# chonlei/neural-ode-ion-channels

Hardware: AMD Instinct MI355X
Metric: trajectories/sec (sinewave protocol, 100k steps) (higher is better)
Workload: dtype f64

## Files before the change

### neural-ode-ion-channels_amd/csrc/ionode_attempt_body.hpp

```cpp
#ifdef IONODE_STAMPS
    constexpr int NET = std::is_same<typename std::decay<decltype(IONODE_NET)>::type, MlpShrink4>::value ? 1 : 0;
    const unsigned long long att0_ = stamp_now();
#endif
    if constexpr (LW) {
#pragma unroll
      for (int i = 0; i < NPAR; ++i) asm volatile("" : "+v"(p[i]));
    }
    bool failed_now = false;
    if (active) {
      if ((int64_t)since >= a.max_steps || (int64_t)nacc + nrej >= a.max_total) { status = IONODE_STATUS_MAX_STEPS; failed_now = true; }
      else if (!(t + dt > t)) { status = IONODE_STATUS_DT_UNDERFLOW; failed_now = true; }
      else {
        bool fin = true;
#pragma unroll
        for (int d = 0; d < D; ++d) fin = fin && isfinite((double)y[d]);
        if (!fin) { status = IONODE_STATUS_NONFINITE; failed_now = true; }
      }
      if (failed_now) active = false;
    }
    {
      unsigned long long fm = __ballot(failed_now && lane < LPS);
      while (fm) {
        const int jj = __builtin_ctzll(fm);
        fm &= fm - 1;
        if (WPS == 1 || (jj % WPS) == wis) {
          const int o0 = __builtin_amdgcn_readlane(oi, jj);
          const int tr = __builtin_amdgcn_readlane(traj, jj);
          S *__restrict__ yo = reinterpret_cast<S *>(a.y_out) + (size_t)tr * Nt * D;
          for (int idx = o0 + lane; idx < Nt && (a.y_out || a.i_out); idx += 64) {
            if (a.y_out) {
#pragma unroll
              for (int d = 0; d < D; ++d) yo[(size_t)idx * D + d] = nan_s;
            }
            if (a.i_out) a.i_out[(size_t)tr * Nt + idx] = __builtin_nan("");
          }
        }
      }
    }
    if constexpr (NSETS > 1) {
      if (__syncthreads_or(active ? 1 : 0) == 0) break;
    } else {
      if (__ballot(active) == 0ull) break;
    }

    const double t0 = t;
    const double t1 = t0 + dt;
    const S dts = (S)dt;
    S k[7][D], yi[D];
#pragma unroll
    for (int d = 0; d < D; ++d) k[0][d] = f[d];
    if constexpr (!CARRY_V) lookup_stages(t0, dt);
    STAMP(stamps_, 1);
    ClosedRates<MT::MLP ? IONODE_MODEL_HH2 : MODEL> cr;
#pragma unroll
    for (int i = 0; i < 6; ++i) {
      S bd[6];
#pragma unroll
      for (int jx = 0; jx <= i; ++jx) bd[jx] = (S)kBeta[i][jx] * dts;
#pragma unroll
      for (int d = 0; d < D; ++d) {
        S s = k[0][d] * bd[0];
#pragma unroll
        for (int jx = 1; jx <= i; ++jx) s = s + k[jx][d] * bd[jx];
        yi[d] = y[d] + s;
      }
      if constexpr (MT::MLP && T64) {
        bool fresh = (i == 0);
        if (i > 0 && i < 5) fresh = __ballot(vst[i] != vst[i > 0 ? i - 1 : 0] || inst[i] != inst[i > 0 ? i - 1 : 0]) != 0ull;
        rhs<MODEL, S, T64>(a, p, vst[i < 4 ? i : 4], inst[i < 4 ? i : 4], yi, k[i + 1], IONODE_NET, &cr, fresh);
      } else if constexpr (MT::MLP) rhs<MODEL, S, T64>(a, p, vst[i < 4 ? i : 4], inst[i < 4 ? i : 4], yi, k[i + 1], IONODE_NET);
      else {
        if (i < 5) {
          bool fresh = (i == 0);
          if (i > 0) fresh = __ballot(vst[i] != vst[i > 0 ? i - 1 : 0] || inst[i] != inst[i > 0 ? i - 1 : 0]) != 0ull;
          if (fresh) closed_rates<MODEL, S>(a, p, vst[i], inst[i], cr);
        }
        closed_rhs<MODEL, S>(cr, yi, k[i + 1]);
      }
    }
    S tmp[D];
    {
      S be[7];
#pragma unroll
      for (int jx = 0; jx < 7; ++jx) be[jx] = dts * (S)kCerr[jx];
#pragma unroll
      for (int d = 0; d < D; ++d) {
        S e = k[0][d] * be[0];
#pragma unroll
        for (int jx = 1; jx < 7; ++jx) e = e + k[jx][d] * be[jx];
        const S ay0 = abs_(y[d]), ay1 = abs_(yi[d]);
        const S tol = atol + rtol * (ay0 > ay1 ? ay0 : ay1);
        tmp[d] = e / tol;
      }
    }
    const S ratio = abs_(rms_norm<S, D>(tmp));
    const bool accept = ratio <= (S)1;

    double dt_next;
    if (ratio == (S)0) dt_next = dt * 10.0;
    else {
      const double dfactor = (ratio < (S)1) ? 1.0 : 0.2;
      const double er = (double)ratio;
      double fac = 0.9 / det_root5(er);
      if (!(fac > dfactor)) fac = dfactor;
      if (!(fac < 10.0)) fac = 10.0;
      if (er != er) fac = __builtin_nan("");
      dt_next = dt * fac;
    }

    STAMP(stamps_, 6);
    const bool acc_now = active && accept;
#ifndef IONODE_STAMPS
    if (a.step_log != nullptr && active && primary && traj_raw == 0 && (int64_t)nacc + nrej < a.step_log_cap) {
      double *row = a.step_log + 4 * ((int64_t)nacc + nrej);
      row[0] = t0; row[1] = dt; row[2] = (double)ratio; row[3] = accept ? 1.0 : 0.0;
    }
#endif
    const int nacc_before = nacc, oi_before = oi;
    if (active) { if (accept) ++nacc; else ++nrej; }
    const double dt_capped = (dt_next > a.dt_max) ? a.dt_max : dt_next;
    if constexpr (CARRY_V) lookup_stages(acc_now ? t1 : t0, (active || acc_now) ? dt_capped : dt);

// ... 420 lines not shown
```

### neural-ode-ion-channels_amd/csrc/ionode_capi.hip

```cpp
#include <algorithm>
#include <cstdio>
#include <cstdlib>
#include <cstring>
#include <vector>

#include "ionode_launch.hpp"

namespace {

constexpr int kTile32From = 8192;
constexpr int kTile4Upto = 1024;
constexpr int kTile1Upto = 256;
constexpr int kTiny64From = 32769;
constexpr int kHh2LaneFrom = 49152;
constexpr int kMarkov6LaneFrom = 24576;

thread_local char g_err[256] = "";
thread_local const char *g_last_kernel = "";

void set_err(const char *fmt, const char *detail = "") { snprintf(g_err, sizeof g_err, fmt, detail); }

inline int np_of(int N) { return 16 * ((N + 15) / 16); }

struct Plan {
// ... 69 lines not shown
  pl->v = find_variant(d->model, d->state_f32 ? 1 : 0, ionode::Net::None, lean, tpw, 1, 0);
  if (!pl->v) { set_err("no kernel variant compiled for this descriptor"); return IONODE_ERR_UNSUPPORTED; }
  plan_lane_wise(pl, (size_t)((d->n_traj + tpw - 1) / tpw), (size_t)ionode::LwLds::bytes(D, pl->v->lds_key));
  return IONODE_OK;
}

int plan_mlp(const ionode_desc *d, Plan *pl, const Ask &k) {
  using ionode::Lean;
  using ionode::Net;
  if (d->mlp_width < 1 || d->mlp_layers < 0) { set_err("bad MLP shape"); return IONODE_ERR_ARG; }
  if (d->mlp_width <= 16 && d->mlp_layers > 10) { set_err("N <= 16 kernels keep at most 10 hidden layers resident"); return IONODE_ERR_UNSUPPORTED; }
  const int f32 = d->state_f32 ? 1 : 0, tw = d->tile_waves, L = d->mlp_layers;
  const int NP = np_of(d->mlp_width), NT = NP / 16;
  if (tw != 0 && tw != 1 && tw != 4 && !(tw == 64 && NT == 1) && !((tw == 8 || tw == 2 || tw == 16) && NT == 13)) {
    set_err("tile_waves must be 0, 1 or 4 for MLP models (64: the N <= 16 kernel at 64 trajectories per wavefront; 8 / 2 / 16: the N = 200 kernel with 32 / 4 / 1 trajectories per tile)");
    return IONODE_ERR_UNSUPPORTED;
  }
  auto images_fill = [&](int tile) { return d->traj_per_image <= 0 || d->traj_per_image % tile == 0; };
  const bool n200 = NT == 13 && L >= 1;
  const bool t64 = NT == 1 && (tw == 64 || (tw == 0 && d->n_traj >= kTiny64From && images_fill(64)));
  const bool vnet = t64 && d->mlp_width == 10;
  const bool t32 = !t64 && n200 && images_fill(32) && (tw == 8 || (tw == 0 && d->n_traj >= kTile32From));
  const bool t1 = !t64 && !t32 && n200 && L <= 15 && (tw == 16 || (tw == 0 && d->n_traj <= kTile1Upto));
  const bool t1deep = t1 && L > ionode::MlpRow1::max_layers();
  const bool t4 = !t64 && !t32 && !t1 && n200 && images_fill(4) && (tw == 2 || (tw == 0 && d->n_traj <= kTile4Upto));
  const bool lean_tile = L >= 1 && no_side_outputs(d, k) && has_exact_grid(d);
  const bool lean_t64 = t64 && has_exact_grid(d) && !k.want_current && no_side_outputs(d, k);
  const bool lean_tuned = !t64 && (NT == 13 || NT == 7 || NT == 32) && lean_tile;
  const Net net = vnet ? Net::Lane : t1 ? (t1deep ? Net::Row1Deep : Net::Row1) : t4 ? Net::Tile4 : Net::Tile;
  const int tpt = t64 ? 64 : t32 ? 32 : t1 ? 1 : t4 ? 4 : 16;
  const int G = t64 ? 1 : ((tw == 8 || tw == 2 || tw == 16) ? 4 : tw);
  pl->v = find_variant(d->model, f32, net, lean_t64 ? Lean::States : (lean_tuned ? Lean::Tile : Lean::General), tpt, G, NT);
  if (!pl->v && NT >= 2 && NT <= ionode::MlpGen::NT_MAX && (tw == 0 || tw == 4)) {
    pl->v = find_variant(d->model, f32, Net::Gen, lean_tile ? Lean::Tile : Lean::General, 16, 4, 0);
    if (pl->v && pl->v->lds_bytes(L, NT) > 160 * 1024) {
      set_err("this (layers, width) needs more than 160 KB of LDS for its biases and activations");
      return IONODE_ERR_UNSUPPORTED;
    }
  }
  if (!pl->v) {
    set_err("MLP width outside the compiled kernel variants: 1 <= N <= 512 (tuned tiles for N = 10, 100, 200, 500 -- architectures "
            "s00-s11 -- and the run-time-width tile for every other N; tile_waves must be 0 or 4 for the latter)");
    return IONODE_ERR_UNSUPPORTED;
  }
  const ionode::Variant *v = pl->v;
  const size_t tiles = (size_t)((d->n_traj + v->traj_per_tile - 1) / v->traj_per_tile);
  pl->grid = (unsigned)tiles;
  pl->block = 64u * v->G;
  pl->lds = v->lds_bytes(L, NT);
  if (v->shrink) {
    const char *ts = getenv("IONODE_TILE_SHRINK");
    pl->tile_shrink = ts == nullptr || ts[0] == '\0' || atoi(ts) != 0;
    pl->lds = std::max(pl->lds, ionode::MlpTile4::lds_bytes(L));
  }
  if (v->lane_wise) plan_lane_wise(pl, tiles, ((pl->lds + 15) & ~(size_t)15) + (size_t)ionode::LwLds::bytes(2, v->lds_key));
  if (d->traj_per_image > 0) {
    if (d->traj_per_image % v->traj_per_tile != 0 || d->mlp_image_stride < (int64_t)ionode_mlp_packed_floats(L, d->mlp_width)) {
      set_err("traj_per_image must be a multiple of the tile size (16; 64 with tile_waves = 64; 32 with tile_waves = 8) and mlp_image_stride at least one packed image");
      return IONODE_ERR_ARG;
    }
  }
  return IONODE_OK;
}

struct DeferPlan {
  int64_t cap = 0, bytes = 0;
};
DeferPlan plan_defer(const ionode_desc *d, const Plan &pl, bool want_i) {
  DeferPlan p;
  if (!pl.v->defer || d->sse_out != nullptr || d->n_state != 2) return p;
  const char *sw = getenv("IONODE_DEFER_DENSE");
  if (sw != nullptr && sw[0] != '\0' && atoi(sw) == 0) return p;
  using Rec = ionode::DenseRecord<2>;
  const int64_t B = d->n_traj, Nt = d->n_out;
  const char *fc = getenv("IONODE_DEFER_DENSE_CAP");
  int64_t cap = (fc != nullptr && fc[0] != '\0') ? atoll(fc) : 0;
  const bool forced = cap > 0;
  if (!forced) {
    const int64_t out_bytes = B * Nt * 2 * (d->state_f32 ? 4 : 8) + (want_i ? B * Nt * 8 : 0);
    cap = (out_bytes / 4) / (B * Rec::BYTES);
  }
  cap = std::min<int64_t>(cap, Nt - 1);
  if (cap < (forced ? 1 : 64)) return p;
  p.cap = cap;
  p.bytes = (int64_t)Rec::workspace_bytes(B, cap);
  return p;
}

constexpr int64_t kDeferTailEighths = 5;
struct TailPlan {
  int64_t rank = 0, fill = 0;
};
TailPlan plan_tail(const Plan &pl, const DeferPlan &dp) {
  TailPlan t;
  t.fill = dp.cap;
  if (dp.cap < 2) return t;
  const int64_t tiles = (int64_t)pl.grid;
  t.rank = tiles * kDeferTailEighths / 8;
  const char *fr = getenv("IONODE_DEFER_TAIL_RANK");
  if (fr != nullptr && fr[0] != '\0') t.rank = std::max<int64_t>(0, std::min<int64_t>(atoll(fr), tiles));
  const char *sw = getenv("IONODE_DEFER_TAIL");
  if (sw != nullptr && sw[0] != '\0') {
    if (strcmp(sw, "all") == 0) t.rank = tiles;
    else if (atoi(sw) == 0) t.rank = 0;
  }
  if (t.rank > 0) t.fill = dp.cap - 1;
// ... 407 lines not shown
```

### neural-ode-ion-channels_amd/csrc/ionode_device.hpp

```cpp
#pragma once

#include <hip/hip_runtime.h>
#include <stdint.h>

#include <type_traits>

#include "../../include/ionode.h"
#include "ionode_form.hpp"
#include "ionode_kargs.hpp"
#include "ionode_math.hpp"
#include "ionode_interp.hpp"
#include "ionode_dense_expand.hpp"

namespace ionode {

struct LwLds {
  static __host__ __device__ constexpr int rowb(int D) { return interp_row_doubles(D) * 8; }
  static __host__ __device__ constexpr int aux_off(int D) { return 64 * rowb(D); }
  static __host__ __device__ constexpr int aux_bytes(int tail) { return (tail == 1 && IONODE_LEAN) ? 0 : 64 * 64; }
  static __host__ __device__ constexpr int owp_off(int D, int tail) { return aux_off(D) + aux_bytes(tail); }
  static __host__ __device__ constexpr int trl_off(int D, int tail) { return owp_off(D, tail) + 256; }
  static __host__ __device__ constexpr int clist_off(int D, int tail) { return trl_off(D, tail) + 256; }
  static __host__ __device__ constexpr int bytes(int D, int tail) { return clist_off(D, tail) + 1024; }
};
static_assert(LwLds::bytes(2, 1) <= 10240 && LwLds::bytes(2, 0) <= 12800 && LwLds::bytes(2, 2) <= 12800, "2-state kernels: 16 / 12 wavefronts per compute unit");

}

#include "ionode_mlp_tile.hpp"
#include "ionode_mlp_tile4.hpp"
#include "ionode_mlp_row1.hpp"
#include "ionode_mlp_lane.hpp"
#include "ionode_mlp_gen.hpp"
#include "ionode_rhs.hpp"

namespace ionode {

template <typename S, int D> __device__ __forceinline__ void store_state(S *dst, const S *v) {
  if constexpr (D == 2 && sizeof(S) == 8) {
    *reinterpret_cast<double2 *>(dst) = make_double2(v[0], v[1]);
  } else if constexpr (D == 2 && sizeof(S) == 4) {
    *reinterpret_cast<float2 *>(dst) = make_float2(v[0], v[1]);
  } else if constexpr (sizeof(S) == 8) {
#pragma unroll
    for (int d = 0; d < D; d += 2) *reinterpret_cast<double2 *>(dst + d) = make_double2(v[d], v[d + 1]);
  } else {
#pragma unroll
    for (int d = 0; d < D; d += 2) *reinterpret_cast<float2 *>(dst + d) = make_float2(v[d], v[d + 1]);
  }
}

template <int MODEL, typename S, int G, int RT, int NT, int PD, int TAIL>
__global__ void __launch_bounds__((KernelForm<MODEL, G, RT, NT, PD, TAIL>::block_threads), (KernelForm<MODEL, G, RT, NT, PD, TAIL>::waves_per_simd)) ionode_dopri5_kernel(const KArgs a_in) {
  using MT = ModelTraits<MODEL>;
  using F = KernelForm<MODEL, G, RT, NT, PD, TAIL>;
  constexpr bool LEAN = IONODE_LEAN && F::lean == Lean::States;
  constexpr bool LEANT = IONODE_LEAN && F::lean == Lean::Table;
  constexpr bool LEANM = IONODE_LEAN && F::lean == Lean::Tile;
  KArgs a = a_in;
  if constexpr (LEANM) a.te_exact = 1;
  if constexpr (LEAN || LEANT || LEANM) { a.prot_t = nullptr; a.step_log = nullptr; a.step_log_cap = 0; a.ckpt = nullptr; a.ckpt_cap = 0; }
  if constexpr (LEAN) { a.i_out = nullptr; a.sse_out = nullptr; a.sse_ref = nullptr; a.v_tab = nullptr; a.te_exact = 1; }
#ifdef IONODE_STAMPS
  a.step_log = a_in.step_log; a.step_log_cap = a_in.step_log_cap;
#endif
  using R = Real<S>;
  constexpr int D = MT::D, NPAR = MT::NPAR;
  constexpr bool T64 = F::t64, LW = F::lane_wise;
  constexpr int NSETS = F::nsets, WPS = G / NSETS;
  constexpr int TPW = F::traj_per_tile, LPS = F::lanes_per_set;

  extern __shared__ __attribute__((aligned(16))) unsigned char smem[];

  const int lane = threadIdx.x & 63;
  const int wgw = __builtin_amdgcn_readfirstlane(threadIdx.x >> 6);
  const int wave = LW ? 0 : wgw;
  const int tile = LW ? (int)((blockIdx.x & 7u) + 8u * ((blockIdx.x >> 3) * (unsigned)IONODE_LW_TILES_PER_WG + (unsigned)wgw)) : (int)blockIdx.x;
  unsigned char *const smem_t = LW ? smem + (size_t)wgw * (size_t)a.lw_bytes : smem;
  if constexpr (LW) {
    if (tile * TPW >= a_in.B) return;
  }
  const int j = lane % LPS;
  const int cset = (NSETS > 1) ? wave / WPS : 0, wis = wave % WPS;
  const bool primary = (lane < LPS) && (wis == 0);
  const int slot_raw = tile * TPW + cset * LPS + j;
  const bool valid = slot_raw < a.B;
// ... 92 lines not shown
  auto te_at = [&](int idx) -> double { return a.te_t0 + (double)idx * a.te_dt; };

  double sse = 0.0;
  if (valid && primary) {
    if (a.y_out) store_state<S, D>(yout, y);
    if (iout) {
      double v0;
      protocol_v(a, pv, t, v0);
      iout[0] = obs_current<S, D>(a, y, v0);
    }
  }
  if (a.sse_out != nullptr && valid) {
    double v0;
    protocol_v(a, pv, t, v0);
    const double r0 = obs_current<S, D>(a, y, v0) - a.sse_ref[(size_t)pidx * Nt];
    sse = r0 * r0;
  }

  int oi = 1;
  int nacc = 0, nrej = 0;
  int since = 0;
  [[maybe_unused]] int nrec = 0;
  int status = IONODE_STATUS_OK;
  bool active = valid && Nt > 1;
  const S nan_s = (S)__builtin_nan("");

  double vst[5];
  bool inst[5];
  auto lookup_stages = [&](double tt, double dd) {
    const S tts = (S)tt, dds = (S)dd, tt1s = (S)(tt + dd);
    if (((MT::MLP && G > 1) || (!MT::MLP && (D > 2 || !VTAB))) && a.prot_t == nullptr) {
      double tq[5], lo[5], hi[5];
      int ix[5];
#pragma unroll
      for (int i = 0; i < 5; ++i) {
        tq[i] = (double)((i >= 4) ? R::prev_(tt1s) : tts + (S)kAlpha[i] * dds);
        inst[i] = protocol_index(a, tq[i], ix[i]);
      }
#pragma unroll
      for (int i = 0; i < 5; ++i) { lo[i] = pv[ix[i] - 1]; hi[i] = pv[ix[i]]; }
#pragma unroll
      for (int i = 0; i < 5; ++i) vst[i] = inst[i] ? protocol_from(a, lo[i], hi[i], ix[i], tq[i]) : a.v_oob;
      return;
    }
#pragma unroll
    for (int i = 0; i < 5; ++i) {
      const S ti = (i >= 4) ? R::prev_(tt1s) : tts + (S)kAlpha[i] * dds;
      inst[i] = protocol_v(a, pv, (double)ti, vst[i]);
    }
  };
  constexpr bool CARRY_V = (LW && D == 2) || (LW && D > 2 && LEAN) || (MT::MLP && G == 1);
  if constexpr (CARRY_V) lookup_stages(t, dt);

  constexpr bool SHRINK = F::shrink;
#ifdef IONODE_STAMPS
  unsigned long long att_cyc[2] = {0, 0}, att_n[2] = {0, 0};
#endif

  auto live_slots = [&]() { return (unsigned)__ballot(active) & 0xffffu; };
  bool more = true;
  if (!SHRINK || !a.tile_shrink || __builtin_popcount(live_slots()) > 4) {
    more = false;
    for (;;) {
#define IONODE_NET mlp
#include "ionode_attempt_body.hpp"
#undef IONODE_NET
      if constexpr (SHRINK) {
        if (a.tile_shrink && __builtin_popcount(live_slots()) <= 4) { more = true; break; }
      }
    }
  }
  if constexpr (SHRINK) {
    const unsigned live = live_slots();
    if (more && live != 0u) {
      asm volatile("s_waitcnt vmcnt(0) lgkmcnt(0)" ::: "memory");
      __syncthreads();
      MlpShrink4 net4;
      net4.init(a, smem_t, wave, lane, tile * TPW, live);
#ifdef IONODE_STAMPS
      net4.t4.sp = &stamps_;
#endif
      for (;;) {
#define IONODE_NET net4
#include "ionode_attempt_body.hpp"
#undef IONODE_NET
      }
    }
  }

#ifdef IONODE_STAMPS
  STAMP(stamps_, 0);
  if (blockIdx.x == 0 && threadIdx.x == 0 && a.step_log != nullptr && a.step_log_cap >= 4)
    for (int i_ = 0; i_ < 16; ++i_) a.step_log[i_] = (double)stamps_.acc[i_];
  if (threadIdx.x == 0 && a.step_log != nullptr) {
    if (blockIdx.x == 0 && a.step_log_cap >= 9) {
      a.step_log[32] = (double)att_cyc[0]; a.step_log[33] = (double)att_n[0];
      a.step_log[34] = (double)att_cyc[1]; a.step_log[35] = (double)att_n[1];
    }
    if (4 * a.step_log_cap >= 64 + (int64_t)gridDim.x) a.step_log[64 + blockIdx.x] = (double)att_n[1];
  }
#ifdef IONODE_ASM_STAMPS
  if constexpr (MT::MLP && G == 4 && NT == 13) {
    unsigned sv_;
    asm volatile("v_accvgpr_read_b32 %0, a92" : "=v"(sv_));
    if (blockIdx.x == 0 && threadIdx.x < 16 && a.step_log != nullptr && a.step_log_cap >= 8) a.step_log[16 + threadIdx.x] = (double)sv_;
  }
// ... 59 lines not shown
```

### neural-ode-ion-channels_amd/csrc/ionode_form.hpp

```cpp
#pragma once

#include <type_traits>

#include "../../include/ionode.h"

#ifndef IONODE_LEAN
#define IONODE_LEAN 1
#endif
#ifndef IONODE_T64_WAVES
#define IONODE_T64_WAVES 1
#endif
#define IONODE_LW_TILES_PER_WG 4

namespace ionode {

template <int MODEL> struct ModelTraits {
  static constexpr int D = (MODEL == IONODE_MODEL_MARKOV6) ? 6 : 2;
  static constexpr int NPAR = (MODEL == IONODE_MODEL_MARKOV6) ? 12 : 8;
  static constexpr bool MLP = (MODEL == IONODE_MODEL_NNF || MODEL == IONODE_MODEL_NND);
};

template <int G, int RT, int NT, int PD, int NSETS> struct MlpTile;
struct MlpTile4;
template <int MRES_> struct MlpRow1T;
using MlpRow1 = MlpRow1T<2>;
using MlpRow1Deep = MlpRow1T<0>;
template <int N> struct MlpLane;
struct MlpGen;
struct NoMlp;

enum class Net { None, Tile, Tile4, Row1, Row1Deep, Lane, Gen };
enum class Lean { General, States, Table, Tile };

template <int MODEL, int G, int RT, int NT, int PD, int TAIL> struct KernelForm {
  static constexpr bool mlp = ModelTraits<MODEL>::MLP;
  static constexpr bool t64 = mlp && RT == 64;
  static constexpr bool lane_wise = !mlp || t64;
  static constexpr int nsets = (mlp && G > 1 && (TAIL & 4)) ? 2 : 1;
  static constexpr Net net = !mlp                                      ? Net::None
                             : (t64 && PD > 1)                         ? Net::Lane
                             : (G == 4 && NT == 13 && (TAIL & 32))     ? ((TAIL & 64) ? Net::Row1Deep : Net::Row1)
                             : (G == 4 && NT == 13 && (TAIL & 16))     ? Net::Tile4
                             : (G == 4 && NT == 0)                     ? Net::Gen
                                                                       : Net::Tile;
  static constexpr Lean lean = lane_wise ? (TAIL == 1 ? Lean::States : ((!mlp && TAIL == 2) ? Lean::Table : Lean::General))
                                         : ((G > 1 && (TAIL & 8)) ? Lean::Tile : Lean::General);
  static constexpr int lanes_per_set = !mlp ? (RT > 0 ? RT : 64) : t64 ? 64 : (net == Net::Row1 || net == Net::Row1Deep) ? 1 : net == Net::Tile4 ? 4 : 16;
  static constexpr int traj_per_tile = lanes_per_set * nsets;
  static constexpr int lds_key = lean == Lean::States ? 1 : (lean == Lean::Table ? 2 : 0);
  static constexpr int block_threads = 64 * (lane_wise ? IONODE_LW_TILES_PER_WG : G);
  static constexpr int waves_per_simd = t64 ? IONODE_T64_WAVES : (MODEL == IONODE_MODEL_HH2 ? 2 : 1);
  static constexpr bool shrink = net == Net::Tile && G == 4 && NT == 13 && PD == 13 && TAIL == 8;
  static constexpr bool defer = shrink;

  using Tile = MlpTile<G, (t64 ? 1 : (RT > 0 ? RT : 1)), (NT > 0 ? NT : 1), ((PD > 0 && net != Net::Lane) ? PD : 1), nsets>;
  using Mlp = std::conditional_t<net == Net::None, NoMlp,
              std::conditional_t<net == Net::Lane, MlpLane<(net == Net::Lane ? PD : 10)>,
              std::conditional_t<net == Net::Row1, MlpRow1,
              std::conditional_t<net == Net::Row1Deep, MlpRow1Deep,
              std::conditional_t<net == Net::Tile4, MlpTile4,
              std::conditional_t<net == Net::Gen, MlpGen, Tile>>>>>>;

  static_assert(mlp || G == 1, "closed-form models use one wavefront per tile");
  static_assert(!t64 || (G == 1 && NT == 1), "64 trajectories per wavefront is the resident-weights (N <= 16) path");
  static_assert(nsets == 1 || net == Net::Tile, "the 4- and one-trajectory tiles have one column set");
};

}
```

### neural-ode-ion-channels_amd/csrc/ionode_launch.hpp

```cpp
#pragma once
#include "ionode_device.hpp"

namespace ionode {

using LaunchFn = hipError_t (*)(const KArgs &, unsigned grid, size_t lds, hipStream_t);

struct Variant {
  int model, f32;
  int G;
  int NT;
  Net net;
  Lean lean;
  int traj_per_tile;
  int lds_key;
  bool lane_wise, shrink;
  bool defer;
  size_t (*lds_bytes)(int L, int NT);
  LaunchFn fn;
  const char *name;
};

template <typename F> size_t net_lds_bytes(int L, int NT) {
  if constexpr (F::net == Net::None) return 0;
  else if constexpr (F::net == Net::Gen) return F::Mlp::lds_bytes(L, NT);
  else if constexpr (F::net == Net::Tile) return F::Mlp::lds_total(L);
  else return F::Mlp::lds_bytes(L);
}

template <int MODEL, typename S, int G, int RT, int NT, int PD, int TAIL>
hipError_t launch(const KArgs &a, unsigned grid, size_t lds, hipStream_t s) {
  using F = KernelForm<MODEL, G, RT, NT, PD, TAIL>;
  auto kern = ionode_dopri5_kernel<MODEL, S, G, RT, NT, PD, TAIL>;
  if constexpr (F::lane_wise) {
    const size_t need = (size_t)LwLds::bytes(ModelTraits<MODEL>::D, F::lds_key);
    if ((size_t)a.lw_bytes < need || (a.lw_bytes & 15) || lds < (size_t)IONODE_LW_TILES_PER_WG * (size_t)a.lw_bytes) return hipErrorInvalidValue;
  }
  if (lds > 64 * 1024) {
    hipError_t e = hipFuncSetAttribute(reinterpret_cast<const void *>(kern),
                                       hipFuncAttributeMaxDynamicSharedMemorySize, (int)lds);
    if (e != hipSuccess) return e;
  }
  hipLaunchKernelGGL(kern, dim3(grid), dim3(F::block_threads), lds, s, a);
  return hipGetLastError();
}

template <int MODEL, typename S, int F32, int G, int RT, int NT, int PD, int TAIL>
constexpr Variant make_variant(const char *name) {
  using F = KernelForm<MODEL, G, RT, NT, PD, TAIL>;
  return Variant{MODEL, F32, G, NT, F::net, F::lean, F::traj_per_tile, F::lds_key, F::lane_wise, F::shrink, F::defer, &net_lds_bytes<F>,
                 &launch<MODEL, S, G, RT, NT, PD, TAIL>, name};
}

#define IONODE_VARIANT(MODEL, S, F32, G, RT, NT, PD, TAIL) IONODE_VARIANT_(MODEL, S, F32, G, RT, NT, PD, TAIL)
#define IONODE_VARIANT_(MODEL, S, F32, G, RT, NT, PD, TAIL) \
  make_variant<MODEL, S, F32, G, RT, NT, PD, TAIL>("ionode_dopri5_kernel<" #MODEL ", " #S ", " #G ", " #RT ", " #NT ", " #PD ", " #TAIL ">")
#define IONODE_MLP_VARIANTS(MODEL, S, F32)                                                      \
  IONODE_VARIANT(MODEL, S, F32, 1, 1, 1, 1, 0), IONODE_VARIANT(MODEL, S, F32, 4, 4, 7, 7, 0),        \
       \
      IONODE_VARIANT(MODEL, S, F32, 1, 64, 1, 1, 0), IONODE_VARIANT(MODEL, S, F32, 1, 64, 1, 1, 1),      \
            \
      IONODE_VARIANT(MODEL, S, F32, 1, 64, 1, 10, 0), IONODE_VARIANT(MODEL, S, F32, 1, 64, 1, 10, 1),    \
      IONODE_VARIANT(MODEL, S, F32, 4, 4, 13, 13, 0), IONODE_VARIANT(MODEL, S, F32, 4, 8, 32, 4, 0),     \
       \
      IONODE_VARIANT(MODEL, S, F32, 4, 4, 13, 13, 4),                                                     \
       \
      IONODE_VARIANT(MODEL, S, F32, 4, 4, 13, 13, 8), IONODE_VARIANT(MODEL, S, F32, 4, 4, 13, 13, 12),    \
       \
      IONODE_VARIANT(MODEL, S, F32, 4, 4, 13, 13, 16), IONODE_VARIANT(MODEL, S, F32, 4, 4, 13, 13, 24),   \
       \
      IONODE_VARIANT(MODEL, S, F32, 4, 4, 13, 13, 32), IONODE_VARIANT(MODEL, S, F32, 4, 4, 13, 13, 40),   \
       \
      IONODE_VARIANT(MODEL, S, F32, 4, 4, 13, 13, 96), IONODE_VARIANT(MODEL, S, F32, 4, 4, 13, 13, 104),  \
                                                    \
      IONODE_VARIANT(MODEL, S, F32, 4, 4, 7, 7, 8), IONODE_VARIANT(MODEL, S, F32, 4, 8, 32, 4, 8),        \
       \
      IONODE_VARIANT(MODEL, S, F32, 4, 1, 0, 1, 0), IONODE_VARIANT(MODEL, S, F32, 4, 1, 0, 1, 8)

const Variant *variants_closed(int *n);
const Variant *variants_nnf_f64(int *n);
const Variant *variants_nnf_f32(int *n);
const Variant *variants_nnd_f64(int *n);
const Variant *variants_nnd_f32(int *n);

}
```

### neural-ode-ion-channels_amd/csrc/ionode_math.hpp

```cpp
#pragma once
#include <hip/hip_runtime.h>
#include <stdint.h>

namespace ionode {

using f32x4 = __attribute__((ext_vector_type(4))) float;
typedef float f32x2 __attribute__((ext_vector_type(2)));

__device__ constexpr double kAlpha[6] = {1.0 / 5, 3.0 / 10, 4.0 / 5, 8.0 / 9, 1.0, 1.0};
__device__ constexpr double kBeta[6][6] = {
    {1.0 / 5, 0, 0, 0, 0, 0},
    {3.0 / 40, 9.0 / 40, 0, 0, 0, 0},
    {44.0 / 45, -56.0 / 15, 32.0 / 9, 0, 0, 0},
    {19372.0 / 6561, -25360.0 / 2187, 64448.0 / 6561, -212.0 / 729, 0, 0},
    {9017.0 / 3168, -355.0 / 33, 46732.0 / 5247, 49.0 / 176, -5103.0 / 18656, 0},
    {35.0 / 384, 0.0, 500.0 / 1113, 125.0 / 192, -2187.0 / 6784, 11.0 / 84},
};
__device__ constexpr double kCerr[7] = {
    35.0 / 384 - 1951.0 / 21600,       0.0,
    500.0 / 1113 - 22642.0 / 50085,    125.0 / 192 - 451.0 / 720,
    -2187.0 / 6784 - -12231.0 / 42400, 11.0 / 84 - 649.0 / 6300,
    -1.0 / 60.0,
};
__device__ constexpr double kCmid[7] = {
    6025192743.0 / 30085553152.0 / 2,     0.0,
    51252292925.0 / 65400821598.0 / 2,    -2691868925.0 / 45128329728.0 / 2,
    187940372067.0 / 1594534317056.0 / 2, -1776094331.0 / 19743644256.0 / 2,
    11237099.0 / 235043384.0 / 2,
};

__device__ __forceinline__ double pow2i(int k) { return __longlong_as_double((long long)(k + 1023) << 52); }

__device__ __forceinline__ double fma_sc(double p, double r, double c) {
  double d;
  asm("v_fma_f64 %0, %1, %2, %3" : "=v"(d) : "v"(p), "v"(r), "s"(c));
  return d;
}

__device__ __forceinline__ double det_exp(double x) {
  if (x != x) return x;
  if (x > 709.782712893384) return __builtin_inf();
  if (x < -745.1332191019412) return 0.0;
  const double kf = rint(x * 0x1.71547652b82fep+0);
  double r = fma(-kf, 0x1.62e42fee00000p-1, x);
  r = fma(-kf, 0x1.a39ef35793c76p-33, r);
  double p = 1.0 / 6227020800.0;
  p = fma(p, r, 1.0 / 479001600.0);
  p = fma(p, r, 1.0 / 39916800.0);
  p = fma(p, r, 1.0 / 3628800.0);
  p = fma(p, r, 1.0 / 362880.0);
  p = fma(p, r, 1.0 / 40320.0);
  p = fma(p, r, 1.0 / 5040.0);
  p = fma(p, r, 1.0 / 720.0);
  p = fma(p, r, 1.0 / 120.0);
  p = fma(p, r, 1.0 / 24.0);
// ... 39 lines not shown
  p = fma_sc(p, r, 1.0 / 479001600.0);
  p = fma_sc(p, r, 1.0 / 39916800.0);
  p = fma_sc(p, r, 1.0 / 3628800.0);
  p = fma_sc(p, r, 1.0 / 362880.0);
  p = fma_sc(p, r, 1.0 / 40320.0);
  p = fma_sc(p, r, 1.0 / 5040.0);
  p = fma_sc(p, r, 1.0 / 720.0);
  p = fma_sc(p, r, 1.0 / 120.0);
  p = fma_sc(p, r, 1.0 / 24.0);
  p = fma_sc(p, r, 1.0 / 6.0);
  p = fma(p, r, 0.5);
  p = fma(p, r, 1.0);
  p = fma(p, r, 1.0);
  return __builtin_ldexp(p, (int)kf);
}

__device__ __forceinline__ double det_exp_s(double x) {
  const double kf = rint(x * 0x1.71547652b82fep+0);
  double r = fma(-kf, 0x1.62e42fee00000p-1, x);
  r = fma(-kf, 0x1.a39ef35793c76p-33, r);
  double p = 1.0 / 6227020800.0;
  p = fma_sc(p, r, 1.0 / 479001600.0);
  p = fma_sc(p, r, 1.0 / 39916800.0);
  p = fma_sc(p, r, 1.0 / 3628800.0);
  p = fma_sc(p, r, 1.0 / 362880.0);
  p = fma_sc(p, r, 1.0 / 40320.0);
  p = fma_sc(p, r, 1.0 / 5040.0);
  p = fma_sc(p, r, 1.0 / 720.0);
  p = fma_sc(p, r, 1.0 / 120.0);
  p = fma_sc(p, r, 1.0 / 24.0);
  p = fma_sc(p, r, 1.0 / 6.0);
  p = fma(p, r, 0.5);
  p = fma(p, r, 1.0);
  p = fma(p, r, 1.0);
  double e = __builtin_ldexp(p, (int)kf);
  e = (x > 709.782712893384) ? __builtin_inf() : e;
  e = (x < -745.1332191019412) ? 0.0 : e;
  return (x != x) ? x : e;
}

__device__ __forceinline__ double div_by(double a, double b, double rb) {
  const double q0 = a * rb;
  const double r = fma(-b, q0, a);
  const double q1 = fma(r, rb, q0);
  const double aq = __builtin_fabs(q0);
  return (aq > 0.0 && aq < __builtin_inf()) ? q1 : q0;
}

__device__ __forceinline__ double div_pos(double a, double b, double rb) {
  const double q0 = a * rb;
  return fma(fma(-b, q0, a), rb, q0);
}

__device__ __forceinline__ double div_const(double a, double b, double rb) {
  const double q0 = a * rb;
  const double r = fma(-b, q0, a);
  const double q1 = fma(r, rb, q0);
  const double aq = __builtin_fabs(q0);
  return (aq > 0x1p-900 && aq < 0x1p+900) ? q1 : a / b;
}
__device__ __forceinline__ float div_constf(float a, float b, float rb) {
  const float q0 = a * rb;
  const float r = fmaf(-b, q0, a);
  const float q1 = fmaf(r, rb, q0);
  const float aq = __builtin_fabsf(q0);
  return (aq > 0x1p-100f && aq < 0x1p+100f) ? q1 : a / b;
}

__device__ __forceinline__ double det_root5(double x) {
  if (!(x < __builtin_inf()) || !(x > 0.0)) return x;
  unsigned long long u = (unsigned long long)__double_as_longlong(x);
  u = u / 5ull + 0x3325999999999999ull;
  double y = __longlong_as_double((long long)u);
#pragma unroll
  for (int it = 0; it < 7; ++it) {
    const double y2 = y * y;
    const double y4 = y2 * y2;
    y = div_by(4.0 * y + x / y4, 5.0, 0.2);
  }
  return y;
}

template <typename S> struct Real;
template <> struct Real<float> {
  static __device__ __forceinline__ float sqrt_(float x) { return sqrtf(x); }
  static __device__ __forceinline__ float prev_(float x) { return nextafterf(x, x - 1.0f); }
};
template <> struct Real<double> {
  static __device__ __forceinline__ double sqrt_(double x) { return sqrt(x); }
  static __device__ __forceinline__ double prev_(double x) { return nextafter(x, x - 1.0); }
};

#ifdef IONODE_STAMPS
struct Stamps {
  unsigned long long acc[16];
  unsigned long long last;
};
__device__ __forceinline__ unsigned long long stamp_now() {
  unsigned long long t;
  asm volatile("s_memtime %0\n\ts_waitcnt lgkmcnt(0)" : "=s"(t)::"memory");
  return t;
}
#define STAMP_DECL Stamps stamps_; for (int i_ = 0; i_ < 16; ++i_) stamps_.acc[i_] = 0; stamps_.last = stamp_now();
#define STAMP(st, slot) do { __builtin_amdgcn_sched_barrier(0); const unsigned long long n_ = stamp_now(); (st).acc[slot] += n_ - (st).last; (st).last = n_; __builtin_amdgcn_sched_barrier(0); } while (0)
#define MSTAMP(slot) STAMP(*sp, slot)
#else
#define STAMP_DECL
#define STAMP(st, slot) do { } while (0)
#define MSTAMP(slot) do { } while (0)
#endif

__device__ __forceinline__ double bcast_f64(double x, int src) {
  const int lo = __builtin_amdgcn_readlane(__double2loint(x), src);
  const int hi = __builtin_amdgcn_readlane(__double2hiint(x), src);
  return __hiloint2double(hi, lo);
}
__device__ __forceinline__ float bcast_f32(float x, int src) {
  return __int_as_float(__builtin_amdgcn_readlane(__float_as_int(x), src));
}
// ... 39 lines not shown
```

### neural-ode-ion-channels_amd/csrc/ionode_rhs.hpp

```cpp
#pragma once

namespace ionode {

struct NoMlp {
  static constexpr int GW = 1;
  __device__ __forceinline__ float eval(float, float) { return 0.0f; }
};

template <int MODEL> struct ClosedRates {
  static constexpr int NR = (MODEL == IONODE_MODEL_MARKOV6) ? 6 : 4;
  double k[NR];
  float kf[NR];
  bool oob32;
};
template <int MODEL, typename S, bool WIDE = false, typename MLP>
__device__ __forceinline__ void rhs(const KArgs &a, const double *p, double v, bool inrange, const S *y, S *f,
                                    MLP &mlp, ClosedRates<IONODE_MODEL_HH2> *cr = nullptr, bool fresh = true) {
  using MT = ModelTraits<MODEL>;
  constexpr bool F32 = sizeof(S) == 4;

  if constexpr (MODEL == IONODE_MODEL_MARKOV6) {
    if (F32 && !inrange) {
      const float vf = (float)a.v_oob;
      const float a1 = (float)p[0] * det_expf((float)p[1] * vf);
      const float b1 = (float)p[2] * det_expf((float)(-p[3]) * vf);
      const float bh = (float)p[4] * det_expf((float)p[5] * vf);
      const float ah = (float)p[6] * det_expf((float)(-p[7]) * vf);
      const float a2 = (float)p[8] * det_expf((float)p[9] * vf);
      const float b2 = (float)p[10] * det_expf((float)(-p[11]) * vf);
      const float c1 = y[0], c2 = y[1], i_ = y[2], ic1 = y[3], ic2 = y[4], o = y[5];
      f[0] = a1 * c2 + ah * ic1 + b2 * o - (b1 + bh + a2) * c1;
      f[1] = b1 * c1 + ah * ic2 - (a1 + bh) * c2;
      f[2] = a2 * ic1 + bh * o - (b2 + ah) * i_;
      f[3] = a1 * ic2 + bh * c1 + b2 * i_ - (b1 + ah + a2) * ic1;
      f[4] = b1 * ic1 + bh * c2 - (ah + a1) * ic2;
      f[5] = a2 * c1 + ah * i_ - (b2 + bh) * o;
      return;
    }
    const double a1 = p[0] * det_exp(p[1] * v);
    const double b1 = p[2] * det_exp(-p[3] * v);
    const double bh = p[4] * det_exp(p[5] * v);
    const double ah = p[6] * det_exp(-p[7] * v);
    const double a2 = p[8] * det_exp(p[9] * v);
    const double b2 = p[10] * det_exp(-p[11] * v);
    const double c1 = y[0], c2 = y[1], i_ = y[2], ic1 = y[3], ic2 = y[4], o = y[5];
    f[0] = (S)(a1 * c2 + ah * ic1 + b2 * o - (b1 + bh + a2) * c1);
    f[1] = (S)(b1 * c1 + ah * ic2 - (a1 + bh) * c2);
    f[2] = (S)(a2 * ic1 + bh * o - (b2 + ah) * i_);
    f[3] = (S)(a1 * ic2 + bh * c1 + b2 * i_ - (b1 + ah + a2) * ic1);
    f[4] = (S)(b1 * ic1 + bh * c2 - (ah + a1) * ic2);
    f[5] = (S)(a2 * c1 + ah * i_ - (b2 + bh) * o);
    return;
  } else {
    constexpr bool HAS_HH_A = (MODEL == IONODE_MODEL_HH2 || MODEL == IONODE_MODEL_NND);
    const S av = y[0], rv = y[1];
    const bool oob32 = F32 && !inrange;

    float net = 0.0f;
    if constexpr (MT::MLP) {
      const float vf = (float)a.v_oob;
      const float nv = oob32 ? vf / 100.0f : (float)div_const(v, 100.0, 0.01);
      if constexpr (WIDE) net = div_constf(mlp.eval_tiny64(nv, (float)av), 1000.0f, 0.001f);
      else net = div_constf(mlp.eval(nv, (float)av), 1000.0f, 0.001f);
    }

    if (oob32) {
      const float vf = (float)a.v_oob;
      const float af = (float)av, rf = (float)rv;
      const float k3 = (float)p[4] * det_expf((float)p[5] * vf);
      const float k4 = (float)p[6] * det_expf((float)(-p[7]) * vf);
      const float drdt = -k3 * rf + k4 * (1.0f - rf);
      float dadt = 0.0f;
      if constexpr (HAS_HH_A) {
        const float k1 = (float)p[0] * det_expf((float)p[1] * vf);
        const float k2 = (float)p[2] * det_expf((float)(-p[3]) * vf);
        dadt = k1 * (1.0f - af) - k2 * af;
      }
      if constexpr (MT::MLP) dadt = (MODEL == IONODE_MODEL_NND) ? dadt + net : net;
      f[0] = (S)dadt;
      f[1] = (S)drdt;
      return;
    }
    const S one_m_a = (S)1 - av;
    const S one_m_r = (S)1 - rv;
    constexpr bool TIGHT = std::is_same<MLP, MlpTile4>::value || std::is_same<MLP, MlpShrink4>::value || std::is_same<MLP, MlpRow1>::value ||
                           std::is_same<MLP, MlpRow1Deep>::value;
    auto dexp = [](double x) { if constexpr (TIGHT) return det_exp_ldexp(x); else if constexpr (MT::MLP && !WIDE) return det_exp_s(x); else return det_exp(x); };
    double k3, k4, dadt = 0.0;
    if constexpr (MT::MLP && WIDE) {
      constexpr int NX = HAS_HH_A ? 4 : 2;
      double kk[4];
      if (fresh || cr == nullptr) {
        double x[NX], e[NX];
        x[0] = p[5] * v; x[1] = -p[7] * v;
        if constexpr (HAS_HH_A) { x[2] = p[1] * v; x[3] = -p[3] * v; }
        bool in = true;
#pragma unroll
        for (int i = 0; i < NX; ++i) in = in && (__builtin_fabs(x[i]) <= 708.0);
        if (__ballot(!in) == 0ull) {
#pragma unroll
          for (int i = 0; i < NX; ++i) e[i] = det_exp_inrange(x[i]);
        } else {
#pragma unroll
          for (int i = 0; i < NX; ++i) e[i] = det_exp_ldexp(x[i]);
        }
        kk[2] = p[4] * e[0]; kk[3] = p[6] * e[1];
        if constexpr (HAS_HH_A) { kk[0] = p[0] * e[2]; kk[1] = p[2] * e[3]; }
        if (cr != nullptr) {
          cr->k[2] = kk[2]; cr->k[3] = kk[3];
          if constexpr (HAS_HH_A) { cr->k[0] = kk[0]; cr->k[1] = kk[1]; }
        }
      } else {
        kk[2] = cr->k[2]; kk[3] = cr->k[3];
        if constexpr (HAS_HH_A) { kk[0] = cr->k[0]; kk[1] = cr->k[1]; }
      }
      k3 = kk[2]; k4 = kk[3];
      if constexpr (HAS_HH_A) dadt = kk[0] * (double)one_m_a - kk[1] * (double)av;
    } else {
      k3 = p[4] * dexp(p[5] * v);
      k4 = p[6] * dexp(-p[7] * v);
      if constexpr (HAS_HH_A) {
        const double k1 = p[0] * dexp(p[1] * v);
        const double k2 = p[2] * dexp(-p[3] * v);
        dadt = k1 * (double)one_m_a - k2 * (double)av;
      }
    }
    const double drdt = -k3 * (double)rv + k4 * (double)one_m_r;
    if constexpr (MT::MLP) dadt = (MODEL == IONODE_MODEL_NND) ? dadt + (double)net : (double)net;
    f[0] = (S)dadt;
    f[1] = (S)drdt;
  }
}

template <int MODEL, typename S>
__device__ __forceinline__ void closed_rates(const KArgs &a, const double *p, double v, bool inrange, ClosedRates<MODEL> &R) {
  constexpr int NR = ClosedRates<MODEL>::NR;
  R.oob32 = (sizeof(S) == 4) && !inrange;
  if (R.oob32) {
    const float vf = (float)a.v_oob;
#pragma unroll
    for (int i = 0; i < NR; ++i) R.kf[i] = (float)p[2 * i] * det_expf((float)((i & 1) ? -p[2 * i + 1] : p[2 * i + 1]) * vf);
  } else {
    double x[NR];
    bool inr = true;
#pragma unroll
    for (int i = 0; i < NR; ++i) {
      x[i] = ((i & 1) ? -p[2 * i + 1] : p[2 * i + 1]) * v;
      inr = inr && (__builtin_fabs(x[i]) <= 708.0);
    }
    if (__ballot(!inr) == 0ull) {
#pragma unroll
      for (int i = 0; i < NR; ++i) R.k[i] = p[2 * i] * det_exp_inrange(x[i]);
    } else {
#pragma unroll
      for (int i = 0; i < NR; ++i) R.k[i] = p[2 * i] * det_exp_ldexp(x[i]);
    }
  }
}
template <int MODEL, typename S>
__device__ __forceinline__ void closed_rhs(const ClosedRates<MODEL> &R, const S *y, S *f) {
  if constexpr (MODEL == IONODE_MODEL_MARKOV6) {
    if (R.oob32) {
      const float a1 = R.kf[0], b1 = R.kf[1], bh = R.kf[2], ah = R.kf[3], a2 = R.kf[4], b2 = R.kf[5];
      const float c1 = y[0], c2 = y[1], i_ = y[2], ic1 = y[3], ic2 = y[4], o = y[5];
      f[0] = a1 * c2 + ah * ic1 + b2 * o - (b1 + bh + a2) * c1;
      f[1] = b1 * c1 + ah * ic2 - (a1 + bh) * c2;
      f[2] = a2 * ic1 + bh * o - (b2 + ah) * i_;
      f[3] = a1 * ic2 + bh * c1 + b2 * i_ - (b1 + ah + a2) * ic1;
      f[4] = b1 * ic1 + bh * c2 - (ah + a1) * ic2;
      f[5] = a2 * c1 + ah * i_ - (b2 + bh) * o;
// ... 30 lines not shown
```

Before: 12710.

## Precompute per-stage rate constants across idle lanes via LDS stage jobs

For multi-wave MLP kernels where only LPS lanes per set carry trajectories, the exponential rate constants and normalized voltage for all five RK stages are now computed up front. The work is spread across the otherwise idle lanes of the wavefront and handed back through a small per-wave LDS buffer, so each stage reads precomputed values instead of evaluating exponentials serially. The division helper is also changed to take the exact-division fallback only when some lane in the wave needs it, instead of selecting per lane. The cost is extra LDS, a tighter LDS limit check, and wave-wide ballots plus LDS traffic in each step.

```diff
diff --git a/neural-ode-ion-channels_amd/csrc/ionode_attempt_body.hpp b/neural-ode-ion-channels_amd/csrc/ionode_attempt_body.hpp
--- a/neural-ode-ion-channels_amd/csrc/ionode_attempt_body.hpp
+++ b/neural-ode-ion-channels_amd/csrc/ionode_attempt_body.hpp
@@ -50,8 +50,10 @@
 #pragma unroll
     for (int d = 0; d < D; ++d) k[0][d] = f[d];
     if constexpr (!CARRY_V) lookup_stages(t0, dt);
+    if constexpr (SJ) sj.template run<TightNet<typename std::decay<decltype(IONODE_NET)>::type>::value>(vst);
     STAMP(stamps_, 1);
     ClosedRates<MT::MLP ? IONODE_MODEL_HH2 : MODEL> cr;
+    [[maybe_unused]] StageConsts<MODEL> sjc;
 #pragma unroll
     for (int i = 0; i < 6; ++i) {
       S bd[6];
@@ -68,6 +70,9 @@
         bool fresh = (i == 0);
         if (i > 0 && i < 5) fresh = __ballot(vst[i] != vst[i > 0 ? i - 1 : 0] || inst[i] != inst[i > 0 ? i - 1 : 0]) != 0ull;
         rhs<MODEL, S, T64>(a, p, vst[i < 4 ? i : 4], inst[i < 4 ? i : 4], yi, k[i + 1], IONODE_NET, &cr, fresh);
+      } else if constexpr (SJ) {
+        if (i < 5) sj.load(i, sjc);
+        rhs<MODEL, S, T64>(a, p, vst[i < 4 ? i : 4], inst[i < 4 ? i : 4], yi, k[i + 1], IONODE_NET, nullptr, true, &sjc);
       } else if constexpr (MT::MLP) rhs<MODEL, S, T64>(a, p, vst[i < 4 ? i : 4], inst[i < 4 ? i : 4], yi, k[i + 1], IONODE_NET);
       else {
         if (i < 5) {
diff --git a/neural-ode-ion-channels_amd/csrc/ionode_capi.hip b/neural-ode-ion-channels_amd/csrc/ionode_capi.hip
--- a/neural-ode-ion-channels_amd/csrc/ionode_capi.hip
+++ b/neural-ode-ion-channels_amd/csrc/ionode_capi.hip
@@ -145,6 +145,10 @@
     const char *ts = getenv("IONODE_TILE_SHRINK");
     pl->tile_shrink = ts == nullptr || ts[0] == '\0' || atoi(ts) != 0;
     pl->lds = std::max(pl->lds, ionode::MlpTile4::lds_bytes(L));
+  }
+  if (pl->lds + v->stage_jobs_bytes > 160 * 1024) {
+    set_err("this (layers, width) needs more than 160 KB of LDS for its biases and activations");
+    return IONODE_ERR_UNSUPPORTED;
   }
   if (v->lane_wise) plan_lane_wise(pl, tiles, ((pl->lds + 15) & ~(size_t)15) + (size_t)ionode::LwLds::bytes(2, v->lds_key));
   if (d->traj_per_image > 0) {
diff --git a/neural-ode-ion-channels_amd/csrc/ionode_device.hpp b/neural-ode-ion-channels_amd/csrc/ionode_device.hpp
--- a/neural-ode-ion-channels_amd/csrc/ionode_device.hpp
+++ b/neural-ode-ion-channels_amd/csrc/ionode_device.hpp
@@ -32,6 +32,7 @@
 #include "ionode_mlp_row1.hpp"
 #include "ionode_mlp_lane.hpp"
 #include "ionode_mlp_gen.hpp"
+#include "ionode_stage_jobs.hpp"
 #include "ionode_rhs.hpp"
 
 namespace ionode {
@@ -230,6 +231,13 @@
   constexpr bool CARRY_V = (LW && D == 2) || (LW && D > 2 && LEAN) || (MT::MLP && G == 1);
   if constexpr (CARRY_V) lookup_stages(t, dt);
 
+  constexpr bool SJ = F::stage_jobs;
+  [[maybe_unused]] StageJobs<MODEL, (SJ ? LPS : 16)> sj;
+  if constexpr (SJ) {
+    __shared__ __attribute__((aligned(16))) unsigned char sj_rows[F::stage_jobs_bytes];
+    sj.init(p, lane, sj_rows + (size_t)wgw * F::stage_jobs_wave_bytes);
+  }
+
   constexpr bool SHRINK = F::shrink;
 #ifdef IONODE_STAMPS
   unsigned long long att_cyc[2] = {0, 0}, att_n[2] = {0, 0};
diff --git a/neural-ode-ion-channels_amd/csrc/ionode_form.hpp b/neural-ode-ion-channels_amd/csrc/ionode_form.hpp
--- a/neural-ode-ion-channels_amd/csrc/ionode_form.hpp
+++ b/neural-ode-ion-channels_amd/csrc/ionode_form.hpp
@@ -9,6 +9,9 @@
 #endif
 #ifndef IONODE_T64_WAVES
 #define IONODE_T64_WAVES 1
+#endif
+#ifndef IONODE_STAGE_JOBS
+#define IONODE_STAGE_JOBS 1
 #endif
 #define IONODE_LW_TILES_PER_WG 4
 
@@ -53,6 +56,11 @@
   static constexpr bool shrink = net == Net::Tile && G == 4 && NT == 13 && PD == 13 && TAIL == 8;
   static constexpr bool defer = shrink;
 
+  static constexpr bool stage_jobs = IONODE_STAGE_JOBS && mlp && !t64 && G > 1;
+  static constexpr int stage_rates = (MODEL == IONODE_MODEL_NND) ? 4 : 2;
+  static constexpr int stage_jobs_wave_bytes = 5 * lanes_per_set * (stage_rates + 1) * 8;
+  static constexpr int stage_jobs_bytes = stage_jobs ? G * stage_jobs_wave_bytes : 0;
+
   using Tile = MlpTile<G, (t64 ? 1 : (RT > 0 ? RT : 1)), (NT > 0 ? NT : 1), ((PD > 0 && net != Net::Lane) ? PD : 1), nsets>;
   using Mlp = std::conditional_t<net == Net::None, NoMlp,
               std::conditional_t<net == Net::Lane, MlpLane<(net == Net::Lane ? PD : 10)>,
diff --git a/neural-ode-ion-channels_amd/csrc/ionode_launch.hpp b/neural-ode-ion-channels_amd/csrc/ionode_launch.hpp
--- a/neural-ode-ion-channels_amd/csrc/ionode_launch.hpp
+++ b/neural-ode-ion-channels_amd/csrc/ionode_launch.hpp
@@ -16,6 +16,7 @@
   bool lane_wise, shrink;
   bool defer;
   size_t (*lds_bytes)(int L, int NT);
+  size_t stage_jobs_bytes;
   LaunchFn fn;
   const char *name;
 };
@@ -35,7 +36,7 @@
     const size_t need = (size_t)LwLds::bytes(ModelTraits<MODEL>::D, F::lds_key);
     if ((size_t)a.lw_bytes < need || (a.lw_bytes & 15) || lds < (size_t)IONODE_LW_TILES_PER_WG * (size_t)a.lw_bytes) return hipErrorInvalidValue;
   }
-  if (lds > 64 * 1024) {
+  if (lds + (size_t)F::stage_jobs_bytes > 64 * 1024) {
     hipError_t e = hipFuncSetAttribute(reinterpret_cast<const void *>(kern),
                                        hipFuncAttributeMaxDynamicSharedMemorySize, (int)lds);
     if (e != hipSuccess) return e;
@@ -47,7 +48,7 @@
 template <int MODEL, typename S, int F32, int G, int RT, int NT, int PD, int TAIL>
 constexpr Variant make_variant(const char *name) {
   using F = KernelForm<MODEL, G, RT, NT, PD, TAIL>;
-  return Variant{MODEL, F32, G, NT, F::net, F::lean, F::traj_per_tile, F::lds_key, F::lane_wise, F::shrink, F::defer, &net_lds_bytes<F>,
+  return Variant{MODEL, F32, G, NT, F::net, F::lean, F::traj_per_tile, F::lds_key, F::lane_wise, F::shrink, F::defer, &net_lds_bytes<F>, (size_t)F::stage_jobs_bytes,
                  &launch<MODEL, S, G, RT, NT, PD, TAIL>, name};
 }
 
diff --git a/neural-ode-ion-channels_amd/csrc/ionode_math.hpp b/neural-ode-ion-channels_amd/csrc/ionode_math.hpp
--- a/neural-ode-ion-channels_amd/csrc/ionode_math.hpp
+++ b/neural-ode-ion-channels_amd/csrc/ionode_math.hpp
@@ -1,6 +1,8 @@
 #pragma once
 #include <hip/hip_runtime.h>
 #include <stdint.h>
+
+#include "ionode_form.hpp"
 
 namespace ionode {
 
@@ -146,19 +148,47 @@
   return fma(fma(-b, q0, a), rb, q0);
 }
 
-__device__ __forceinline__ double div_const(double a, double b, double rb) {
+__device__ __forceinline__ double div_const_sel(double a, double b, double rb) {
   const double q0 = a * rb;
   const double r = fma(-b, q0, a);
   const double q1 = fma(r, rb, q0);
   const double aq = __builtin_fabs(q0);
   return (aq > 0x1p-900 && aq < 0x1p+900) ? q1 : a / b;
 }
-__device__ __forceinline__ float div_constf(float a, float b, float rb) {
+__device__ __forceinline__ float div_constf_sel(float a, float b, float rb) {
   const float q0 = a * rb;
   const float r = fmaf(-b, q0, a);
   const float q1 = fmaf(r, rb, q0);
   const float aq = __builtin_fabsf(q0);
   return (aq > 0x1p-100f && aq < 0x1p+100f) ? q1 : a / b;
+}
+__device__ __forceinline__ double div_const(double a, double b, double rb) {
+#if IONODE_STAGE_JOBS
+  const double q0 = a * rb;
+  const double r = fma(-b, q0, a);
+  const double q1 = fma(r, rb, q0);
+  const double aq = __builtin_fabs(q0);
+  const bool ok = aq > 0x1p-900 && aq < 0x1p+900;
+  if (__builtin_expect(__ballot(!ok) == 0ull, 1)) return q1;
+  asm volatile("" : "+v"(a));
+  return ok ? q1 : a / b;
+#else
+  return div_const_sel(a, b, rb);
+#endif
+}
+__device__ __forceinline__ float div_constf(float a, float b, float rb) {
+#if IONODE_STAGE_JOBS
+  const float q0 = a * rb;
+  const float r = fmaf(-b, q0, a);
+  const float q1 = fmaf(r, rb, q0);
+  const float aq = __builtin_fabsf(q0);
+  const bool ok = aq > 0x1p-100f && aq < 0x1p+100f;
+  if (__builtin_expect(__ballot(!ok) == 0ull, 1)) return q1;
+  asm volatile("" : "+v"(a));
+  return ok ? q1 : a / b;
+#else
+  return div_constf_sel(a, b, rb);
+#endif
 }
 
 __device__ __forceinline__ double det_root5(double x) {
diff --git a/neural-ode-ion-channels_amd/csrc/ionode_rhs.hpp b/neural-ode-ion-channels_amd/csrc/ionode_rhs.hpp
--- a/neural-ode-ion-channels_amd/csrc/ionode_rhs.hpp
+++ b/neural-ode-ion-channels_amd/csrc/ionode_rhs.hpp
@@ -1,6 +1,11 @@
 #pragma once
 
 namespace ionode {
+
+template <typename MLP> struct TightNet {
+  static constexpr bool value = std::is_same<MLP, MlpTile4>::value || std::is_same<MLP, MlpShrink4>::value || std::is_same<MLP, MlpRow1>::value ||
+                                std::is_same<MLP, MlpRow1Deep>::value;
+};
 
 struct NoMlp {
   static constexpr int GW = 1;
@@ -15,7 +20,8 @@
 };
 template <int MODEL, typename S, bool WIDE = false, typename MLP>
 __device__ __forceinline__ void rhs(const KArgs &a, const double *p, double v, bool inrange, const S *y, S *f,
-                                    MLP &mlp, ClosedRates<IONODE_MODEL_HH2> *cr = nullptr, bool fresh = true) {
+                                    MLP &mlp, ClosedRates<IONODE_MODEL_HH2> *cr = nullptr, bool fresh = true,
+                                    const StageConsts<MODEL> *sc = nullptr) {
   using MT = ModelTraits<MODEL>;
   constexpr bool F32 = sizeof(S) == 4;
 
@@ -59,9 +65,13 @@
     float net = 0.0f;
     if constexpr (MT::MLP) {
       const float vf = (float)a.v_oob;
-      const float nv = oob32 ? vf / 100.0f : (float)div_const(v, 100.0, 0.01);
-      if constexpr (WIDE) net = div_constf(mlp.eval_tiny64(nv, (float)av), 1000.0f, 0.001f);
-      else net = div_constf(mlp.eval(nv, (float)av), 1000.0f, 0.001f);
+      if constexpr (WIDE) {
+        const float nv = oob32 ? vf / 100.0f : (float)div_const_sel(v, 100.0, 0.01);
+        net = div_constf_sel(mlp.eval_tiny64(nv, (float)av), 1000.0f, 0.001f);
+      } else {
+        const float nv = oob32 ? vf / 100.0f : (sc != nullptr ? sc->nv : (float)div_const(v, 100.0, 0.01));
+        net = div_constf(mlp.eval(nv, (float)av), 1000.0f, 0.001f);
+      }
     }
 
     if (oob32) {
@@ -83,8 +93,7 @@
     }
     const S one_m_a = (S)1 - av;
     const S one_m_r = (S)1 - rv;
-    constexpr bool TIGHT = std::is_same<MLP, MlpTile4>::value || std::is_same<MLP, MlpShrink4>::value || std::is_same<MLP, MlpRow1>::value ||
-                           std::is_same<MLP, MlpRow1Deep>::value;
+    constexpr bool TIGHT = TightNet<MLP>::value;
     auto dexp = [](double x) { if constexpr (TIGHT) return det_exp_ldexp(x); else if constexpr (MT::MLP && !WIDE) return det_exp_s(x); else return det_exp(x); };
     double k3, k4, dadt = 0.0;
     if constexpr (MT::MLP && WIDE) {
@@ -116,6 +125,10 @@
       }
       k3 = kk[2]; k4 = kk[3];
       if constexpr (HAS_HH_A) dadt = kk[0] * (double)one_m_a - kk[1] * (double)av;
+    } else if (MT::MLP && sc != nullptr) {
+      constexpr int NR = StageConsts<MODEL>::NR;
+      k3 = sc->k[NR - 2]; k4 = sc->k[NR - 1];
+      if constexpr (HAS_HH_A) dadt = sc->k[0] * (double)one_m_a - sc->k[1] * (double)av;
     } else {
       k3 = p[4] * dexp(p[5] * v);
       k4 = p[6] * dexp(-p[7] * v);
diff --git a/neural-ode-ion-channels_amd/csrc/ionode_stage_jobs.hpp b/neural-ode-ion-channels_amd/csrc/ionode_stage_jobs.hpp
--- /dev/null
+++ b/neural-ode-ion-channels_amd/csrc/ionode_stage_jobs.hpp
@@ -0,0 +1,87 @@
+#pragma once
+
+namespace ionode {
+
+template <int MODEL> struct StageConsts {
+  static constexpr int NR = (MODEL == IONODE_MODEL_NND) ? 4 : 2;
+  double k[NR];
+  float nv;
+};
+
+template <int MODEL, int LPS> struct StageJobs {
+  static constexpr int NR = StageConsts<MODEL>::NR;
+  static constexpr int R = 64 / LPS;
+  static constexpr int J = 5 * NR;
+  static constexpr int PASSES = (J + R - 1) / R;
+  static constexpr int SPP = R / NR;
+  static constexpr int ENTRY = NR + 1;
+  static constexpr int WAVE_BYTES = 5 * LPS * ENTRY * 8;
+  static_assert(R % NR == 0 && 64 % LPS == 0, "a pass covers whole stages");
+
+  double mult, coef;
+  double *mine;
+  const double *slot;
+  int s0;
+  bool first;
+
+  __device__ __forceinline__ void init(const double *p, int lane, unsigned char *row) {
+    const int j = lane % LPS, rho = lane / LPS, e = rho % NR;
+    constexpr int base = (NR == 4) ? 0 : 4;
+    mult = p[base]; coef = p[base + 1];
+#pragma unroll
+    for (int i = 1; i < NR; ++i) {
+      const double c = (i & 1) ? -p[base + 2 * i + 1] : p[base + 2 * i + 1];
+      if (e == i) { mult = p[base + 2 * i]; coef = c; }
+    }
+    s0 = rho / NR;
+    first = (e == 0);
+    double *r = reinterpret_cast<double *>(row);
+    slot = r + j * ENTRY;
+    mine = r + (s0 * LPS + j) * ENTRY + e;
+  }
+
+  template <bool TIGHT> __device__ __forceinline__ void run(const double *vst) {
+    double v[PASSES], x[PASSES], ex[PASSES];
+    bool on[PASSES];
+#pragma unroll
+    for (int m = 0; m < PASSES; ++m) {
+      constexpr int last = 4;
+      const int lo = (m * SPP < last) ? m * SPP : last, hi = (m * SPP + SPP - 1 < last) ? m * SPP + SPP - 1 : last;
+      on[m] = m * SPP + s0 <= last;
+      v[m] = vst[hi];
+#pragma unroll
+      for (int s = 0; s < 5; ++s) {
+        if (s >= lo && s < hi) {
+          double vs = vst[s];
+          asm("" : "+v"(vs));
+          v[m] = (m * SPP + s0 == s) ? vs : v[m];
+        }
+      }
+      x[m] = coef * v[m];
+    }
+#pragma unroll
+    for (int m = 0; m < PASSES; ++m) {
+      if constexpr (TIGHT) ex[m] = det_exp_ldexp(x[m]);
+      else ex[m] = det_exp_s(x[m]);
+    }
+#pragma unroll
+    for (int m = 0; m < PASSES; ++m) {
+      const double kk = mult * ex[m];
+      const float nv = (float)div_const(v[m], 100.0, 0.01);
+      if (on[m]) {
+        double *w = mine + m * (SPP * LPS * ENTRY);
+        *w = kk;
+        if (first) *reinterpret_cast<float *>(w + NR) = nv;
+      }
+    }
+  }
+
+  __device__ __forceinline__ void load(int s, StageConsts<MODEL> &c) const {
+    const double *r = slot + s * (LPS * ENTRY);
+#pragma unroll
+    for (int e = 0; e < NR; ++e) c.k[e] = r[e];
+    c.nv = *reinterpret_cast<const float *>(r + NR);
+  }
+};
+
+}
```

Result: no change. 12760, median of 6 (+0.4%).
